# CESNET/GPUJPEG

Measured on AMD Instinct MI355X. Metric: Mpix/s encode+decode (8K RGB q75), higher is better.
Workload: dtype f32

## Files before the change

gpujpeg_amd/csrc/gj_enc_internal.h:

```cpp
#pragma once
#include <hip/hip_runtime.h>
#include <stdlib.h>

#include "gj_device.h"
#include "gj_hip.h"

#define GJ_ENC_MAX_SPT 64
#define GJ_ASM_SEGS 4

template <int CS_FROM, int CS_TO>
__device__ __forceinline__ void gj_color_static(int& a, int& b, int& c)
{
    if (CS_FROM == CS_TO || CS_FROM == GJ_CS_NONE || CS_TO == GJ_CS_NONE) return;
    if (CS_FROM == GJ_CS_RGB) gj_rgb_to(CS_TO, a, b, c);
    else if (CS_TO == GJ_CS_RGB) gj_to_rgb(CS_FROM, a, b, c);
}

template <int R0 = 0, int R1 = 8>
__device__ __forceinline__ void gj_load_444(const gj_geom& g, const uint8_t* __restrict__ raw, const unsigned bx, const unsigned by, uint32_t (&px)[8][6])
{
    const size_t pitch = (size_t)g.width * 3 + g.width_padding;
    const bool interior = (bx * 8 + 8 <= (unsigned)g.width) && (by * 8 + 8 <= (unsigned)g.height);
    const bool aligned = ((pitch | (size_t)raw) & 3) == 0;
    if (interior && aligned) {
        const uint8_t* row = raw + (size_t)(by * 8 + R0) * pitch + (size_t)bx * 24;
#pragma unroll
        for (int r = R0; r < R1; r++) {
            const uint2* p = reinterpret_cast<const uint2*>(row);
            const uint2 a = p[0], b = p[1], c = p[2];
            px[r][0] = a.x; px[r][1] = a.y; px[r][2] = b.x; px[r][3] = b.y; px[r][4] = c.x; px[r][5] = c.y;
            row += pitch;
        }
    } else {
#pragma unroll
        for (int r = R0; r < R1; r++) {
            const unsigned y = by * 8 + r;
#pragma unroll
            for (int w = 0; w < 6; w++) {
                uint32_t d = 0;
#pragma unroll
                for (int b = 0; b < 4; b++) {
                    const unsigned byte = w * 4 + b, x = bx * 8 + byte / 3;
                    if (x < (unsigned)g.width && y < (unsigned)g.height) d |= (uint32_t)raw[(size_t)y * pitch + (size_t)x * 3 + byte % 3] << (8 * b);
                }
                px[r][w] = d;
            }
        }
    }
}

template <int CS_FROM, int CS_TO>
__device__ __forceinline__ void gj_color_444(const gj_geom& g, const unsigned bx, const unsigned by, const uint32_t (&px)[8][6], uint32_t (&pk)[3][16])
{
    const bool interior = (bx * 8 + 8 <= (unsigned)g.width) && (by * 8 + 8 <= (unsigned)g.height);
#pragma unroll
    for (int r = 0; r < 8; r++) {
        uint32_t o0[2], o1[2], o2[2];
        gj_color_row<CS_FROM, CS_TO>(px[r], o0, o1, o2);
        if (!interior) {
            const int cols = min(8, max(0, g.width - (int)(bx * 8))), rows = min(8, max(0, g.height - (int)(by * 8)));
            const uint32_t m_lo = cols >= 4 ? 0xFFFFFFFFu : (1u << (8 * cols)) - 1u;
            const uint32_t m_hi = cols >= 8 ? 0xFFFFFFFFu : cols > 4 ? (1u << (8 * (cols - 4))) - 1u : 0u;
            const uint32_t lo = r < rows ? m_lo : 0u, hi = r < rows ? m_hi : 0u;
            o0[0] &= lo; o0[1] &= hi; o1[0] &= lo; o1[1] &= hi; o2[0] &= lo; o2[1] &= hi;
        }
        pk[0][r * 2] = o0[0]; pk[0][r * 2 + 1] = o0[1];
        pk[1][r * 2] = o1[0]; pk[1][r * 2 + 1] = o1[1];
        pk[2][r * 2] = o2[0]; pk[2][r * 2 + 1] = o2[1];
        GJ_KEEP6(pk[0][r * 2], pk[0][r * 2 + 1], pk[1][r * 2], pk[1][r * 2 + 1], pk[2][r * 2], pk[2][r * 2 + 1]);
    }
}

template <int CS_FROM, int CS_TO>
__device__ __forceinline__ void gj_load_color_444(const gj_geom& g, const uint8_t* __restrict__ raw, const unsigned bx, const unsigned by, uint32_t (&pk)[3][16])
{
    uint32_t px[8][6];
    gj_load_444(g, raw, bx, by, px);
    gj_color_444<CS_FROM, CS_TO>(g, bx, by, px, pk);
}


typedef uint32_t __attribute__((aligned(1))) gj_u32_unaligned;
struct GjTail {
    uint32_t* piece;
    uint32_t* group;
    uint32_t* group_other;
    uint32_t ngroups, npieces;
    const uint8_t* temp;
    const uint32_t* seg_bytes;
    const uint32_t* seg_ff;
    uint8_t* jpeg;
    uint64_t capacity;
    const uint8_t* scan_hdr;
    uint32_t hdr_end[GJ_MAX_COMP];
    uint32_t scan_first[GJ_MAX_COMP];
    uint32_t seg_first[GJ_MAX_COMP];
    uint32_t segs[GJ_MAX_COMP];
    uint32_t block_first[GJ_MAX_COMP];
    uint32_t spt, seg_blocks;
    uint64_t temp_blocks;
    uint32_t main_hdr;
    uint32_t* d_result;
    uint32_t* h_result;
    uint64_t f_raw, f_temp, f_jpeg;
    uint32_t f_seg, f_tail;
    uint32_t tail_from, tiles;
};

__device__ __forceinline__ uint32_t gj_pick4(const uint32_t (&a)[GJ_MAX_COMP], const uint32_t s)
{
    return s == 0 ? a[0] : s == 1 ? a[1] : s == 2 ? a[2] : a[3];
}
__device__ __forceinline__ uint32_t gj_tail_scan_of(const GjTail& T, const uint32_t p)
{
    return (p >= T.scan_first[1] ? 1u : 0u) + (p >= T.scan_first[2] ? 1u : 0u) + (p >= T.scan_first[3] ? 1u : 0u);
}
__device__ __forceinline__ void gj_piece_put(const GjTail& T, const uint32_t p, const uint32_t size, const size_t frame_words = 0)
{
    T.piece[frame_words + p] = size;
    (void)__hip_atomic_fetch_add(&T.group[frame_words + (p >> 5)], size, __ATOMIC_RELAXED, __HIP_MEMORY_SCOPE_AGENT);
}


typedef void (*gj_fused_kernel_t)(const gj_geom, const uint8_t*, int16_t*, const float*, const float*);
typedef void (*gj_encode_kernel_t)(const gj_geom, const uint8_t*, const float*, const float*, const uint32_t*, uint8_t*, uint32_t*, uint32_t*, const GjTail);
gj_fused_kernel_t gj_fused_kernel(const gj_geom& g);
gj_fused_kernel_t gj_fused_uyvy422_kernel();
gj_encode_kernel_t gj_encode_kernel(const gj_geom& g, const bool one_component = false);
gj_encode_kernel_t gj_encode_uyvy422_kernel();
gj_encode_kernel_t gj_encode_blocks_kernel(const bool planar);
__global__ void k_preprocess(const gj_geom g, const uint8_t* __restrict__ raw, uint8_t* __restrict__ planes);
__global__ void k_copy_planes_in(const gj_geom g, const uint8_t* __restrict__ raw, uint8_t* __restrict__ planes);
__global__ void k_dct(const gj_geom g, const uint8_t* __restrict__ planes, int16_t* __restrict__ coefs, const float* __restrict__ q_luma, const float* __restrict__ q_chroma);
__global__ void k_huffman(const gj_geom g, const int16_t* __restrict__ coefs, const uint32_t* __restrict__ lut, uint8_t* __restrict__ temp, uint32_t* __restrict__ seg_bytes,
                          uint32_t* __restrict__ seg_ff);
__global__ void k_huffman_count(const gj_geom g, const int16_t* __restrict__ coefs, uint32_t* __restrict__ freq);
__global__ void k_gather(const GjTail T0);
__global__ void k_scan_segments(const gj_enc_job J, unsigned long long* __restrict__ partial, const uint32_t epoch);
__global__ void k_assemble(const gj_enc_job J);
__global__ void k_segment_info(const gj_enc_job J);
```

gpujpeg_amd/csrc/gj_enc_tiles.hip:

```cpp
#include "gj_enc_internal.h"

#ifdef GJ_TRACE_PHASES
static __device__ unsigned long long* gj_trace_buf_e;
extern "C" GJ_HIP_API int gj_hip_trace_set_encoder(void* p) { return hipMemcpyToSymbol(HIP_SYMBOL(gj_trace_buf_e), &p, sizeof p) == hipSuccess ? 0 : -1; }
static __device__ int gj_trace_stop_e = 1 << 30;
extern "C" GJ_HIP_API int gj_hip_trace_stop_encoder(int n) { return hipMemcpyToSymbol(HIP_SYMBOL(gj_trace_stop_e), &n, sizeof n) == hipSuccess ? 0 : -1; }
#define GJ_TRACE_E(slot) do { if (threadIdx.x == 0 && gj_trace_buf_e) gj_trace_buf_e[(size_t)blockIdx.x * 16 + (slot)] = __builtin_amdgcn_s_memrealtime(); \
                              if ((slot) >= gj_trace_stop_e) __builtin_amdgcn_endpgm(); } while (0)
#else
#define GJ_TRACE_E(slot) ((void)0)
#endif

#define GJ_ENC_PRIV_ROWS 24
#define GJ_ENC_WIN_DW ((32 - GJ_ENC_PRIV_ROWS) * 256)

__device__ static constexpr uint8_t GJ_IZZ[64] = {0,  1,  5,  6,  14, 15, 27, 28, 2,  4,  7,  13, 16, 26, 29, 42, 3,  8,  12, 17, 25, 30,
                                                  41, 43, 9,  11, 18, 24, 31, 40, 44, 53, 10, 19, 23, 32, 39, 45, 52, 54, 20, 22, 33, 38,
                                                  46, 51, 55, 60, 21, 34, 37, 47, 50, 56, 59, 61, 35, 36, 48, 49, 57, 58, 62, 63};
#define GJ_COL_OFF(z) (((z) & 31) * 1024 + ((z) >> 5) * 2)

__device__ __forceinline__ void gj_fdct_quant_zz(const uint32_t (&px)[16], const float* __restrict__ q, uint8_t* col)
{
    gj_f2 D[8][4];
#pragma unroll
    for (int r = 0; r < 8; r++) {
        const uint32_t a = px[2 * r], b = px[2 * r + 1];
        D[r][0] = gj_f2{gj_ubyte_f_opaque<0>(a), gj_ubyte_f_opaque<1>(a)};
        D[r][1] = gj_f2{gj_ubyte_f_opaque<2>(a), gj_ubyte_f_opaque<3>(a)};
        D[r][2] = gj_f2{gj_ubyte_f_opaque<0>(b), gj_ubyte_f_opaque<1>(b)};
        D[r][3] = gj_f2{gj_ubyte_f_opaque<2>(b), gj_ubyte_f_opaque<3>(b)};
    }
#pragma unroll
    for (int c = 0; c < 4; c++) gj_fdct8<gj_f2>(D[0][c], D[1][c], D[2][c], D[3][c], D[4][c], D[5][c], D[6][c], D[7][c], -1024.0f);
    __builtin_amdgcn_sched_barrier(0);
    const gj_f2* q2 = reinterpret_cast<const gj_f2*>(q);
#pragma unroll
    for (int rp = 0; rp < 4; rp++) {
        gj_f2 E[8];
#pragma unroll
        for (int cp = 0; cp < 4; cp++) {
            E[2 * cp] = gj_f2{D[2 * rp][cp].x, D[2 * rp + 1][cp].x};
            E[2 * cp + 1] = gj_f2{D[2 * rp][cp].y, D[2 * rp + 1][cp].y};
        }
        gj_fdct8<gj_f2>(E[0], E[1], E[2], E[3], E[4], E[5], E[6], E[7], 0.0f);
#pragma unroll
        for (int j = 0; j < 8; j++) {
            const gj_f2 u = E[j] * q2[j * 4 + rp] + (gj_f2)12582912.0f;
            const float fx = u.x, fy = u.y;
            *reinterpret_cast<uint16_t*>(col + GJ_COL_OFF(GJ_IZZ[(2 * rp) * 8 + j])) = (uint16_t)__builtin_bit_cast(uint32_t, fx);
            *reinterpret_cast<uint16_t*>(col + GJ_COL_OFF(GJ_IZZ[(2 * rp + 1) * 8 + j])) = (uint16_t)__builtin_bit_cast(uint32_t, fy);
        }
        __builtin_amdgcn_sched_barrier(0);
    }
}

struct GjCoderLds {
    uint32_t* coef;
    const uint32_t* lut;
    uint32_t* wsum;
    int* edge;
    uint32_t *segx, *segend, *segbase, *segbits, *segff;
};

struct GjWalk {
    uint32_t hi;
    int room;
    int produced;
    int stored;
    int lim;
};
#define GJ_ENC_NO_STORE 4096

__device__ __forceinline__ void gj_put(GjWalk& w, const uint32_t cw, const int n, uint8_t* col, uint32_t* __restrict__ spill, const int p)
{
    w.room -= n;
    const uint64_t t = (uint64_t)cw << w.room;
    w.hi |= (uint32_t)(t >> 32);
    if (w.room <= 32) {
        if (w.lim <= min(p, GJ_ENC_PRIV_ROWS - 1)) {
            *reinterpret_cast<uint16_t*>(col + w.produced * 2048) = (uint16_t)(w.hi >> 16);
            *reinterpret_cast<uint16_t*>(col + w.produced * 2048 + 1024) = (uint16_t)w.hi;
            w.lim += 2;
        } else {
            if (w.lim != GJ_ENC_NO_STORE) w.stored = w.produced;
            spill[w.produced] = w.hi;
            w.lim = GJ_ENC_NO_STORE;
        }
        w.produced++;
        w.hi = (uint32_t)t;
        w.room += 32;
    }
}

template <bool NONZERO>
__device__ __forceinline__ void gj_value_bits2(const int v, int& nbits, uint32_t& bits)
{
    const int s = v >> 31, t = v + s;
    if (NONZERO) {
        nbits = 32 - gj_ffbh_i32(t);
    } else {
        const uint32_t a = (uint32_t)(t ^ s) | 1u;
        nbits = v ? 32 - __builtin_clz(a) : 0;
    }
    bits = __builtin_amdgcn_ubfe((uint32_t)t, 0, (uint32_t)nbits);
}

__device__ __forceinline__ void gj_walk_ac(uint8_t* col, const uint32_t mlo, const uint32_t mhi, const uint32_t* lut_ac, GjWalk& w,
                                           uint32_t* __restrict__ spill)
{
    int prev = 0;
#pragma unroll
    for (int half = 0; half < 2; half++) {
        uint32_t m = half ? mhi : mlo;
        while (m) {
            const int b = __builtin_ctz(m), p = b + 32 * half;
            m &= m - 1;
            int run = p - prev - 1;
            prev = p;
            const int v = *reinterpret_cast<const int16_t*>(col + b * 1024 + half * 2);
            if (run >= 16) {
                const uint32_t zrl = lut_ac[0xF0];
                do {
                    gj_put(w, zrl & 0x03FFFFFFu, (int)(zrl >> 26), col, spill, p);
                    run -= 16;
                } while (run >= 16);
            }
            const int sg = v >> 31, t = v + sg, k = gj_ffbh_i32(t);
            const uint32_t bits = __builtin_amdgcn_ubfe((uint32_t)t, 0, (uint32_t)(32 - k));
            const uint32_t ent = (lut_ac - 16)[gj_lshl_add_u32<4>((uint32_t)run, (uint32_t)k)];
            gj_put(w, (ent & 0x03FFFFFFu) | bits, (int)(ent >> 26), col, spill, p);
        }
    }
    if (prev != 63) {
        const uint32_t eob = lut_ac[0];
        gj_put(w, eob & 0x03FFFFFFu, (int)(eob >> 26), col, spill, 63);
    }
}

template <bool WHOLE>
__device__ __forceinline__ void gj_merge_stream(const GjWalk& w, const uint8_t* col, const uint32_t* __restrict__ spill, const uint64_t tail,
                                                const int ndw, const uint32_t sh, const uint32_t d0, uint32_t* s_bits, const uint32_t wbase,
                                                const uint32_t wend)
{
    uint32_t prevv = 0, d = d0;
    auto emit = [&](const uint32_t cur) {
        const uint32_t out = __builtin_amdgcn_alignbit(prevv, cur, sh);
        if (out && (WHOLE || (d >= wbase && d < wend))) atomicOr(&s_bits[d - wbase], out);
        prevv = cur;
        d++;
    };
    const int stored = w.lim == GJ_ENC_NO_STORE ? w.stored : w.produced;
    for (int f = 0; f < stored; f++)
        emit(((uint32_t)*reinterpret_cast<const uint16_t*>(col + f * 2048) << 16) | *reinterpret_cast<const uint16_t*>(col + f * 2048 + 1024));
    for (int f = stored; f < w.produced; f++) emit(spill[f]);
    emit((uint32_t)(tail >> 32));
    if (ndw > w.produced) emit((uint32_t)tail);
    if (ndw > w.produced + 1) emit(0u);
}

__device__ __forceinline__ uint32_t gj_code_tile(const GjCoderLds& L, const int i, const int j, const int k, const bool active, const int spt,
                                                 const int nblocks, const int table, const int dc_dist, const int seg_count_left,
                                                 uint8_t* __restrict__ region,
                                                 uint32_t* __restrict__ seg_bytes, uint32_t* __restrict__ seg_ff, const uint32_t first_segment,
                                                 const int trace0 = -1)
{
    (void)trace0;
    const int lane = i & 63, wave = i >> 6;
    uint8_t* const col = reinterpret_cast<uint8_t*>(L.coef) + i * 4;
    uint32_t* const s_bits = L.coef + GJ_ENC_PRIV_ROWS * 256;
    const uint32_t* const lut_ac = L.lut + table * 272;
    const uint32_t* const lut_dc = lut_ac + 256;

    uint32_t mlo = 0, mhi = 0;
    int dc = 0;
    {
        uint32_t elo = 0, ehi = 0;
#pragma unroll
        for (int q = 0; q < 32; q++) {
            const uint32_t d = L.coef[q * 256 + i];
            if (q == 0) dc = (int)(int16_t)(d & 0xFFFFu);
            const uint32_t m = gj_pk_min_u16(d, 0x00010001u);
            if (q < 16) elo |= m << q;
            else ehi |= m << (q - 16);
        }
        if (active) {
            mlo = __builtin_amdgcn_perm(ehi, elo, 0x05040100u);
            mhi = __builtin_amdgcn_perm(ehi, elo, 0x07060302u);
        }
    }
    if (lane >= 48) L.edge[wave * 16 + (lane - 48)] = dc;
    if (i < GJ_ENC_MAX_SPT) L.segff[i] = 0;
    __syncthreads();

    GjWalk w = {0, 64, 0, 0, 1};
    uint32_t* const spill = reinterpret_cast<uint32_t*>(region + (size_t)i * GJ_TEMP_BYTES_PER_BLOCK);
    int dc_diff = 0;
    {
        const int src = lane - dc_dist;
        int pred = __builtin_amdgcn_ds_bpermute((src & 63) << 2, dc);
        if (src < 0 && wave > 0) pred = L.edge[(wave - 1) * 16 + (16 + src)];
        if (k - dc_dist < 0) pred = 0;
        dc_diff = dc - pred;
    }
    if (active) {
        int nbits;
        uint32_t bits;
        gj_value_bits2<false>(dc_diff, nbits, bits);
        const uint32_t ent = lut_dc[nbits];
        gj_put(w, (ent & 0x03FFFFFFu) | bits, (int)(ent >> 26), col, spill, 0);
        gj_walk_ac(col, mlo & ~1u, mhi, lut_ac, w, spill);
    }
    const int fill = 64 - w.room;
    const uint32_t len = (uint32_t)w.produced * 32u + (uint32_t)fill;

    if (trace0 >= 0) GJ_TRACE_E(trace0 + 1);
    const uint32_t winc = gj_wave_incl_scan(len);
    if (lane == 63) L.wsum[wave] = winc;
    __syncthreads();
    uint32_t excl;
    {
        const uint32_t a = L.wsum[0], b = L.wsum[1], c = L.wsum[2];
        const uint32_t incl = winc + (wave == 0 ? 0u : wave == 1 ? a : wave == 2 ? a + b : a + b + c);
        if (active && k == 0) L.segx[j] = incl - len;
        if (active && k == nblocks - 1) L.segend[j] = incl;
        excl = incl - len;
    }
    {
        uint4* z = reinterpret_cast<uint4*>(s_bits) + i * 2;
        z[0] = make_uint4(0, 0, 0, 0);
        z[1] = make_uint4(0, 0, 0, 0);
    }
    __syncthreads();
    if (trace0 >= 0) GJ_TRACE_E(trace0 + 2);
    uint32_t sbits = 0, sdw = 0;
    if (lane < spt && lane < seg_count_left) {
        sbits = L.segend[lane] - L.segx[lane];
        sbits += (8u - (sbits & 7u)) & 7u;
        sdw = (sbits + 31u) >> 5;
    }
    const uint32_t sbase_incl = gj_wave_incl_scan(sdw);
    const uint32_t sbase = sbase_incl - sdw;
    const uint32_t total_dw = (uint32_t)__builtin_amdgcn_readlane((int)sbase_incl, 63);
    if (wave == 0) {
        if (lane < spt) { L.segbase[lane] = sbase; L.segbits[lane] = sbits; }
        if (lane == 63) L.segbase[spt] = total_dw;
    }
    uint32_t start_bit = 0;
    int pad_bits = 0;
    {
        const uint32_t my_base = (uint32_t)__builtin_amdgcn_ds_bpermute(j << 2, (int)sbase);
        const uint32_t my_x = active ? L.segx[j] : 0u;
        start_bit = my_base * 32u + (excl - my_x);
        if (active && k == nblocks - 1) pad_bits = (int)((8u - ((start_bit + len) & 7u)) & 7u);
    }

    const uint32_t sh = start_bit & 31u, d0 = start_bit >> 5;
    uint64_t tail = (uint64_t)w.hi << 32;
    if (pad_bits) tail |= (uint64_t)((1u << pad_bits) - 1u) << (64 - fill - pad_bits);
    const int ndw = w.produced + (fill + pad_bits > 32 ? 2 : (fill + pad_bits > 0 ? 1 : 0));
    const int nseg = min(spt, seg_count_left);
    uint32_t* const dst = reinterpret_cast<uint32_t*>(region);
    for (uint32_t wbase = 0; wbase < total_dw; wbase += GJ_ENC_WIN_DW) {
        const uint32_t wend = min(total_dw, wbase + (uint32_t)GJ_ENC_WIN_DW);
        if (wbase) {
            __syncthreads();
            for (uint32_t d = i; d < wend - wbase; d += 256) s_bits[d] = 0;
            __syncthreads();
        }
        if (active && d0 + (uint32_t)ndw + 1u > wbase && d0 < wend) {
            if (total_dw <= (uint32_t)GJ_ENC_WIN_DW) gj_merge_stream<true>(w, col, spill, tail, ndw, sh, d0, s_bits, 0u, total_dw);
            else gj_merge_stream<false>(w, col, spill, tail, ndw, sh, d0, s_bits, wbase, wend);
        }
        __syncthreads();
        for (int sl = wave; sl < nseg; sl += 4) {
            const uint32_t sb = L.segbase[sl], nfl = (L.segbits[sl] + 31u) >> 5;
            const uint32_t lo = max(sb, wbase), hi = min(sb + nfl, wend);
            uint32_t ffc = 0;
            for (uint32_t d = lo + (uint32_t)lane; d < hi; d += 64) {
                const uint32_t v = s_bits[d - wbase];
                ffc += (uint32_t)__builtin_popcount(((v & 0x7F7F7F7Fu) + 0x01010101u) & v & 0x80808080u);
                dst[d] = __builtin_bswap32(v);
            }
            ffc = gj_wave_incl_scan(ffc);
            if (lane == 63 && ffc) L.segff[sl] += ffc;
        }
    }
    __syncthreads();
    if (trace0 >= 0) GJ_TRACE_E(trace0 + 3);
    uint32_t out = 0;
    if (lane < nseg) {
        const uint32_t nb = (L.segbits[lane] + 7u) >> 3, ff = L.segff[lane];
        out = nb + ff + (lane != seg_count_left - 1 ? 2u : 0u);
        if (wave == 0) {
            seg_bytes[first_segment + lane] = nb;
            seg_ff[first_segment + lane] = ff;
        }
    }
    return (uint32_t)__builtin_amdgcn_readlane((int)gj_wave_incl_scan(out), 63);
}

__device__ __forceinline__ void gj_load_coder_lut(uint32_t* s_lut, const uint32_t* __restrict__ lut, const int i)
{
    static_assert(GJ_CODER_LUT_WORDS == 2 * 272 && GJ_CODER_LUT_WORDS % 4 == 0, "layout of GjCoderLds::lut");
    if (i < GJ_CODER_LUT_WORDS / 4) reinterpret_cast<uint4*>(s_lut)[i] = reinterpret_cast<const uint4*>(lut + GJ_CODER_LUT_OFFSET)[i];
}


template <int CS_FROM, int CS_TO, bool ONE_COMPONENT = false>
__global__ __launch_bounds__(256, 4) void k_encode_rgb444(const gj_geom g, const uint8_t* __restrict__ raw, const float* __restrict__ q_luma,
                                                          const float* __restrict__ q_chroma, const uint32_t* __restrict__ lut,
                                                          uint8_t* __restrict__ temp, uint32_t* __restrict__ seg_bytes,
                                                          uint32_t* __restrict__ seg_ff, const GjTail T)
{
    __shared__ __attribute__((aligned(16))) uint32_t s_coef[32 * 256];
    __shared__ __attribute__((aligned(8))) float s_q[3][64];
    __shared__ __attribute__((aligned(16))) uint32_t s_lut[2 * 272];
    __shared__ uint32_t s_wsum[4];
    __shared__ int s_edge[64];
    __shared__ uint32_t s_segx[GJ_ENC_MAX_SPT], s_segend[GJ_ENC_MAX_SPT], s_segbase[GJ_ENC_MAX_SPT + 1], s_segbits[GJ_ENC_MAX_SPT], s_segff[GJ_ENC_MAX_SPT];
    const GjCoderLds L = {s_coef, s_lut, s_wsum, s_edge, s_segx, s_segend, s_segbase, s_segbits, s_segff};

    const int i = threadIdx.x;
    GJ_TRACE_E(0);
    gj_load_coder_lut(s_lut, lut, i);
    if (i < 192) s_q[i >> 6][i & 63] = (g.comp[i >> 6].type ? q_chroma : q_luma)[i & 63];
    const size_t fz = blockIdx.z;
    raw += fz * T.f_raw;
    temp += fz * T.f_temp;
    seg_bytes += fz * T.f_seg;
    seg_ff += fz * T.f_seg;

    const gj_comp_geom& k0 = g.comp[0];
    const int B = g.seg_blocks;
    const int spt = 256 / B;
    const int tile_blocks = spt * B;
    const uint32_t recip = (65536u + (uint32_t)B - 1u) / (uint32_t)B;
    const int j = min((int)(((uint32_t)i * recip) >> 16), GJ_ENC_MAX_SPT - 1);
    const int k = i - j * B;
    unsigned tile = blockIdx.x, ntiles = gridDim.x;
    int only = ONE_COMPONENT ? (int)blockIdx.y : -1;
    if (!ONE_COMPONENT && T.tail_from != 0xFFFFFFFFu) {
        ntiles = T.tiles;
        if (blockIdx.x >= T.tail_from) {
            const unsigned r = blockIdx.x - T.tail_from, q = r / 3u;
            tile = T.tail_from + q;
            only = (int)(r - 3u * q);
        }
    }
    const int seg0 = (int)tile * spt;
    const unsigned nb = (unsigned)(k0.blocks_x * k0.blocks_y);
    const unsigned lb = tile * (unsigned)tile_blocks + (unsigned)i;
    const bool active = i < tile_blocks && lb < nb;
    unsigned bx, by;
    {
        const unsigned bxn = (unsigned)k0.blocks_x, lbc = min(lb, nb - 1u);
        if (bxn >= 256u) {
            const unsigned lb0 = tile * (unsigned)tile_blocks;
            const unsigned by0 = (unsigned)__builtin_amdgcn_readfirstlane((int)(lb0 / bxn));
            bx = lbc - by0 * bxn;
            by = by0;
            if (bx >= bxn) { bx -= bxn; by++; }
        } else {
            by = lbc / bxn;
            bx = lbc - by * bxn;
        }
    }

    uint32_t pk[3][16];
    gj_load_color_444<CS_FROM, CS_TO>(g, raw, bx, by, pk);
    __syncthreads();
    GJ_TRACE_E(1);

#pragma unroll
    for (int c = 0; c < 3; c++) {
        if (only >= 0 && c != only) continue;
        const gj_comp_geom& kc = g.comp[c];
#pragma unroll
        for (int t = 0; t < 16; t++) GJ_KEEP(pk[c][t]);
        gj_fdct_quant_zz(pk[c], s_q[c], reinterpret_cast<uint8_t*>(s_coef) + i * 4);
        GJ_TRACE_E(2 + 4 * c);
        const uint64_t first_block = kc.data_offset / 64 + (uint64_t)seg0 * B;
        const uint32_t size = gj_code_tile(L, i, j, k, active, spt, active ? min(B, (int)nb - (seg0 + j) * B) : 0, kc.type, 1, k0.segment_count - seg0,
                                           temp + first_block * GJ_TEMP_BYTES_PER_BLOCK, seg_bytes, seg_ff, (uint32_t)(kc.first_segment + seg0), 2 + 4 * c);
        if (i == 0) gj_piece_put(T, (uint32_t)c * ntiles + tile, size, fz * T.f_tail);
    }
}

__global__ __launch_bounds__(256, 4) void k_encode_uyvy422(const gj_geom g, const uint8_t* __restrict__ raw, const float* __restrict__ q_luma,
                                                           const float* __restrict__ q_chroma, const uint32_t* __restrict__ lut,
                                                           uint8_t* __restrict__ temp, uint32_t* __restrict__ seg_bytes,
                                                           uint32_t* __restrict__ seg_ff, const GjTail T)
{
    __shared__ __attribute__((aligned(16))) uint32_t s_coef[32 * 256];
    __shared__ __attribute__((aligned(8))) float s_q[2][64];
    __shared__ __attribute__((aligned(16))) uint32_t s_lut[2 * 272];
    __shared__ uint32_t s_wsum[4];
    __shared__ int s_edge[64];
    __shared__ uint32_t s_segx[GJ_ENC_MAX_SPT], s_segend[GJ_ENC_MAX_SPT], s_segbase[GJ_ENC_MAX_SPT + 1], s_segbits[GJ_ENC_MAX_SPT], s_segff[GJ_ENC_MAX_SPT];
    const GjCoderLds L = {s_coef, s_lut, s_wsum, s_edge, s_segx, s_segend, s_segbase, s_segbits, s_segff};

    const int i = threadIdx.x;
    gj_load_coder_lut(s_lut, lut, i);
    if (i < 128) s_q[i >> 6][i & 63] = (i < 64 ? q_luma : q_chroma)[i & 63];
    raw += (size_t)blockIdx.z * T.f_raw;
    temp += (size_t)blockIdx.z * T.f_temp;
    seg_bytes += (size_t)blockIdx.z * T.f_seg;
    seg_ff += (size_t)blockIdx.z * T.f_seg;

    const gj_comp_geom& kc = g.comp[1];
    const int ri = g.restart_interval;
    const int B = g.seg_blocks;
    const int spt = 256 / B;
    const int tile_blocks = spt * B;
    const uint32_t recip = (65536u + (uint32_t)B - 1u) / (uint32_t)B;
    const int j = min((int)(((uint32_t)i * recip) >> 16), GJ_ENC_MAX_SPT - 1);
    const int k = i - j * B;
    const int p = k & 3;
    const int seg0 = blockIdx.x * spt;
    const unsigned m = (unsigned)(seg0 + j) * (unsigned)ri + (unsigned)(k >> 2);
    const unsigned nm = (unsigned)g.mcu_count;
    const bool active = i < tile_blocks && seg0 + j < g.segment_count && m < nm;
    const unsigned my = m / (unsigned)kc.blocks_x, mx = m - my * (unsigned)kc.blocks_x;

    uint32_t px[16];
    {
        const size_t pitch = (size_t)g.width * 2 + g.width_padding;
        const bool interior = (mx * 16 + 16 <= (unsigned)g.width) && (my * 8 + 8 <= (unsigned)g.height);
        const bool aligned = ((pitch | (size_t)raw) & 15) == 0;
        if (!active) {
#pragma unroll
            for (int t = 0; t < 16; t++) px[t] = 0;
        } else if (interior && aligned) {
            const uint4* src = reinterpret_cast<const uint4*>(raw + (size_t)(my * 8) * pitch + (size_t)mx * 32);
            const size_t pitch4 = pitch >> 4;
            const int first = p == 1;
            const uint32_t selc = p == 2 ? 0x05040100u : 0x07060302u;
            uint4 lo[8], hi[8];
#pragma unroll
            for (int r = 0; r < 8; r++) {
                lo[r] = src[r * pitch4 + first];
                hi[r] = src[r * pitch4 + 1];
            }
#pragma unroll
            for (int r = 0; r < 8; r++) {
                const uint32_t y0 = __builtin_amdgcn_perm(lo[r].y, lo[r].x, 0x07050301u), y1 = __builtin_amdgcn_perm(lo[r].w, lo[r].z, 0x07050301u);
                const uint32_t uv01 = __builtin_amdgcn_perm(lo[r].y, lo[r].x, 0x06020400u), uv23 = __builtin_amdgcn_perm(lo[r].w, lo[r].z, 0x06020400u);
                const uint32_t uv45 = __builtin_amdgcn_perm(hi[r].y, hi[r].x, 0x06020400u), uv67 = __builtin_amdgcn_perm(hi[r].w, hi[r].z, 0x06020400u);
                const uint32_t c0 = __builtin_amdgcn_perm(uv23, uv01, selc), c1 = __builtin_amdgcn_perm(uv67, uv45, selc);
                px[2 * r] = p < 2 ? y0 : c0;
                px[2 * r + 1] = p < 2 ? y1 : c1;
            }
        } else {
#pragma unroll
            for (int r = 0; r < 8; r++) {
                const unsigned y = my * 8 + r;
                uint32_t d[2] = {0, 0};
#pragma unroll
                for (int t = 0; t < 8; t++) {
                    uint32_t v = 0;
                    if (y < (unsigned)g.height) {
                        if (p < 2) {
                            const unsigned x = mx * 16 + p * 8 + t;
                            if (x < (unsigned)g.width) v = raw[(size_t)y * pitch + (size_t)x * 2 + 1];
                        } else {
                            const unsigned cx = mx * 8 + t;
                            if (cx < (unsigned)kc.width) v = raw[(size_t)y * pitch + (size_t)cx * 4 + (p == 2 ? 0 : 2)];
// ... 223 lines not shown
```

gpujpeg_amd/csrc/gj_encode.hip:

```cpp
#include "gj_enc_internal.h"

static GjTail gj_make_tail(const gj_enc_job* job, const unsigned pieces, const unsigned (&scan_first)[GJ_MAX_COMP], const unsigned spt)
{
    const gj_geom& g = job->g;
    GjTail T;
    for (int s = 0; s < GJ_MAX_COMP; s++) {
        T.scan_first[s] = scan_first[s];
        T.hdr_end[s] = job->scan_hdr_offset[s + 1];
        const bool own_scan = !g.interleaved && s < g.comp_count;
        T.seg_first[s] = own_scan ? (uint32_t)g.comp[s].first_segment : 0u;
        T.segs[s] = own_scan ? (uint32_t)g.comp[s].segment_count : (uint32_t)g.segment_count;
        T.block_first[s] = own_scan ? (uint32_t)(g.comp[s].data_offset / 64) : 0u;
    }
    T.spt = spt;
    T.seg_blocks = (uint32_t)g.seg_blocks;
    const unsigned ngcap = GJ_TAIL_GROUPS_CAP(g.segment_count);
    T.group = job->d_tail + (job->tail_set & 1) * ngcap;
    T.group_other = job->d_tail + ((job->tail_set + 1) & 1) * ngcap;
    T.ngroups = (pieces + 31) / 32;
    T.piece = job->d_tail + 2 * ngcap;
    T.npieces = pieces;
    T.temp = job->d_temp;
    T.temp_blocks = (uint64_t)g.block_count;
    T.seg_bytes = job->d_seg_bytes;
    T.seg_ff = job->d_seg_ff;
    T.jpeg = job->d_jpeg;
    T.capacity = job->jpeg_capacity;
    T.scan_hdr = job->d_scan_hdr;
    T.main_hdr = job->main_hdr_size;
    T.d_result = job->d_result;
    T.h_result = job->h_result;
    const bool batch = job->batch.count > 1;
    T.f_raw = batch ? job->batch.raw : 0;
    T.f_temp = batch ? job->batch.temp : 0;
    T.f_jpeg = batch ? job->batch.jpeg : 0;
    T.f_seg = batch ? job->batch.seg : 0;
    T.f_tail = batch ? job->batch.tail : 0;
    return T;
}


static int gj_blocks_kernel_mode(const gj_geom& g)
{
    if (g.no_transform) return 1;
    if (g.pixel_format != GJ_PF_444_P012 || g.comp_count != 3) return -1;
    const int from = g.color_space, to = g.color_space_internal;
    const bool none = from == to || from == GJ_CS_NONE || to == GJ_CS_NONE;
    if (!none && !(from == GJ_CS_RGB && (to == GJ_CS_BT601 || to == GJ_CS_BT601_256 || to == GJ_CS_BT709))) return -1;
    return 0;
}

static bool gj_is_uyvy_layout(const gj_enc_job* job)
{
    const gj_geom& g = job->g;
    return job->use_fused && g.pixel_format == GJ_PF_422_P1020 && g.comp_count == 3 && g.no_transform == 0 &&
           (g.color_space == g.color_space_internal || g.color_space == GJ_CS_NONE || g.color_space_internal == GJ_CS_NONE) &&
           g.comp[0].samp_h == 2 && g.comp[0].samp_v == 1 && g.comp[1].samp_h == 1 && g.comp[1].samp_v == 1 && g.comp[2].samp_h == 1 &&
           g.comp[2].samp_v == 1 && g.comp[0].blocks_x == 2 * g.comp[1].blocks_x && g.comp[0].blocks_y == g.comp[1].blocks_y &&
           g.comp[2].blocks_x == g.comp[1].blocks_x && g.comp[2].blocks_y == g.comp[1].blocks_y;
}
static int gj_tile_kernel(const gj_enc_job* job)
{
    const gj_geom& g = job->g;
    if (job->stage != GJ_ENC_STAGE_ALL) return 0;
    const bool segs_ok = g.restart_interval > 0 && g.seg_blocks <= 256 && g.seg_blocks >= 256 / GJ_ENC_MAX_SPT;
    gj_encode_kernel_t whole = (job->use_fused && !job->keep_coefs) ? gj_encode_kernel(g) : nullptr;
    if (whole && job->tune.enc_by_blocks > 0 && gj_blocks_kernel_mode(g) == 0) whole = nullptr;
    if (gj_is_uyvy_layout(job) && !job->keep_coefs && g.interleaved && segs_ok && g.blocks_per_mcu == 4 && g.mcu_count == g.comp[1].blocks_x * g.comp[1].blocks_y &&
        g.comp[1].type == g.comp[2].type && !job->tune.enc_no_whole422)
        return 1;
    if (!whole && job->use_fused && !job->keep_coefs && segs_ok && gj_blocks_kernel_mode(g) >= 0) return 2;
    return whole ? 3 : 0;
}

extern "C" int gj_hip_encode_batchable(const gj_enc_job* job)
{
    return job->use_fused && !job->keep_coefs && !job->channel_remap && !job->flipped && !job->segment_info && gj_tile_kernel(job) != 0;
}

extern "C" int gj_hip_encode_tiles(const gj_enc_job* job) { return gj_tile_kernel(job) != 0; }

extern "C" int gj_hip_encode(const gj_enc_job* job, gj_stream_t stream, gj_event_t ev[GJ_ENC_EVENTS])
{
    hipStream_t st = (hipStream_t)stream;
    const gj_geom& g = job->g;
    if (g.blocks_per_mcu > GJ_MAX_MCU_BLOCKS) return -1;
    const unsigned frames = job->batch.count > 1 ? job->batch.count : 1u;
    if (frames > 1 && (!gj_hip_encode_batchable(job) || frames > 65535u)) return -1;
    if (job->stage != GJ_ENC_STAGE_ALL && (frames > 1 || (job->stage == GJ_ENC_STAGE_COUNT && !job->d_huff_freq))) return -1;
    gj_hip_note_reset();
    const bool code_only = job->stage == GJ_ENC_STAGE_CODE;
    if (ev && !code_only) GJ_HIP_CHECK(hipEventRecord((hipEvent_t)ev[0], st));
    if (job->channel_remap && !code_only) {
        const unsigned n = (unsigned)g.width * (unsigned)g.height;
        hipLaunchKernelGGL(k_channel_remap, dim3((n + 255) / 256), dim3(256), 0, st, g, const_cast<uint8_t*>(job->d_raw), job->channel_remap & 0xFFFFu);
    }
    bool tiles = true;
    GjTail T;
    T.npieces = 0;
    const int tile_kernel = gj_tile_kernel(job);
    gj_encode_kernel_t whole = tile_kernel == 3 ? gj_encode_kernel(g) : nullptr;
    gj_fused_kernel_t fused = job->use_fused ? gj_fused_kernel(g) : nullptr;
    const bool uyvy = gj_is_uyvy_layout(job);
    if (tile_kernel == 1) {
        if (ev) GJ_HIP_CHECK(hipEventRecord((hipEvent_t)ev[1], st));
        if (ev) GJ_HIP_CHECK(hipEventRecord((hipEvent_t)ev[2], st));
        const int spt = 256 / g.seg_blocks;
        const unsigned wgs = ((unsigned)g.segment_count + spt - 1) / spt;
        T = gj_make_tail(job, wgs, {0u, ~0u, ~0u, ~0u}, (unsigned)spt);
        hipLaunchKernelGGL(gj_encode_uyvy422_kernel(), dim3(wgs, 1, frames), dim3(256), 0, st, g, job->d_raw, job->d_fwd_q[0], job->d_fwd_q[1], job->d_huff_lut,
                           job->d_temp, job->d_seg_bytes, job->d_seg_ff, T);
    } else if (tile_kernel == 2) {
        if (ev) GJ_HIP_CHECK(hipEventRecord((hipEvent_t)ev[1], st));
        if (ev) GJ_HIP_CHECK(hipEventRecord((hipEvent_t)ev[2], st));
        const int spt = 256 / g.seg_blocks;
        unsigned wgs = 0, scan_first[GJ_MAX_COMP] = {0u, ~0u, ~0u, ~0u};
        if (g.interleaved) wgs = ((unsigned)g.segment_count + spt - 1) / spt;
        else
            for (int c = 0; c < g.comp_count; c++) {
                scan_first[c] = wgs;
// ... 81 lines not shown
```

gpujpeg_amd/csrc/gj_runtime.hip:

```cpp
#include <hip/hip_runtime.h>
#include <stdlib.h>
#include <string.h>

#include <cstdio>
#include <cstring>
#include <mutex>

#include "gj_hip.h"

static thread_local hipError_t g_last = hipSuccess;

static int chk(hipError_t e)
{
    if (e != hipSuccess) {
        g_last = e;
        return -1;
    }
    return 0;
}

extern "C" {

int gj_hip_note(int hip_error) { return chk((hipError_t)hip_error); }
void gj_hip_note_reset(void) { g_last = hipSuccess; }
// ... 87 lines not shown
static hipStream_t g_lane[64][2];
static int g_lanes_enabled = 1;
static void gj_lanes_forget(int dev)
{
    std::lock_guard<std::mutex> lk(g_lane_mutex);
    if (dev >= 0 && dev < 64) g_lane[dev][0] = g_lane[dev][1] = nullptr;
}
static hipStream_t gj_lane(int dir, size_t n)
{
    int dev = 0;
    if (hipGetDevice(&dev) != hipSuccess || dev < 0 || dev >= 64) return nullptr;
    std::lock_guard<std::mutex> lk(g_lane_mutex);
    if (!g_lanes_enabled || n < g_lane_min_bytes) return nullptr;
    if (!g_lane[dev][dir] && hipStreamCreateWithFlags(&g_lane[dev][dir], hipStreamNonBlocking) != hipSuccess) {
        (void)hipGetLastError();
        g_lane[dev][dir] = nullptr;
    }
    return g_lane[dev][dir];
}
int gj_hip_upload(void* d, const void* s, size_t n, gj_stream_t st, gj_event_t done)
{
    hipStream_t lane = done ? gj_lane(0, n) : nullptr;
    if (!lane) return chk(hipMemcpyAsync(d, s, n, hipMemcpyHostToDevice, (hipStream_t)st));
    if (chk(hipMemcpyAsync(d, s, n, hipMemcpyHostToDevice, lane)) || chk(hipEventRecord((hipEvent_t)done, lane))) return -1;
    return chk(hipEventSynchronize((hipEvent_t)done));
}
int gj_hip_download(void* d, const void* s, size_t n, gj_stream_t st, gj_event_t done)
{
    hipStream_t lane = done ? gj_lane(1, n) : nullptr;
    if (!lane) return chk(hipMemcpyAsync(d, s, n, hipMemcpyDeviceToHost, (hipStream_t)st));
    if (chk(hipStreamSynchronize((hipStream_t)st))) return -1;
    if (chk(hipMemcpyAsync(d, s, n, hipMemcpyDeviceToHost, lane)) || chk(hipEventRecord((hipEvent_t)done, lane))) return -1;
    return chk(hipEventSynchronize((hipEvent_t)done));
}
gj_stream_t gj_hip_lane_begin(int download, size_t bytes_each, gj_stream_t st)
{
    hipStream_t lane = gj_lane(download ? 1 : 0, bytes_each);
    if (!lane) return st;
    if (download && chk(hipStreamSynchronize((hipStream_t)st))) return st;
    return (gj_stream_t)lane;
}
int gj_hip_lane_end(gj_stream_t lane, gj_stream_t st, gj_event_t done)
{
    if (lane == st) return 0;
    if (chk(hipEventRecord((hipEvent_t)done, (hipStream_t)lane))) return -1;
    return chk(hipEventSynchronize((hipEvent_t)done));
}
int gj_hip_memset(void* d, int v, size_t n, gj_stream_t st) { return chk(hipMemsetAsync(d, v, n, (hipStream_t)st)); }
int gj_hip_stream_sync(gj_stream_t st) { return chk(hipStreamSynchronize((hipStream_t)st)); }

int gj_hip_is_device_ptr(const void* p)
{
    hipPointerAttribute_t a;
    std::memset(&a, 0, sizeof a);
    if (hipPointerGetAttributes(&a, p) != hipSuccess) {
        (void)hipGetLastError();
        return 0;
    }
    return a.type == hipMemoryTypeDevice ? 1 : 0;
}

gj_event_t gj_hip_event_create(void)
{
    hipEvent_t e = nullptr;
    if (chk(hipEventCreate(&e))) return nullptr;
    return (gj_event_t)e;
}
void gj_hip_event_destroy(gj_event_t e)
{
    if (e) (void)hipEventDestroy((hipEvent_t)e);
}
int gj_hip_event_record(gj_event_t e, gj_stream_t s) { return chk(hipEventRecord((hipEvent_t)e, (hipStream_t)s)); }
float gj_hip_event_elapsed_ms(gj_event_t a, gj_event_t b)
{
    float ms = 0.0f;
    if (hipEventSynchronize((hipEvent_t)b) != hipSuccess) return 0.0f;
    if (hipEventElapsedTime(&ms, (hipEvent_t)a, (hipEvent_t)b) != hipSuccess) return 0.0f;
    return ms;
}

}

static std::mutex g_tune_mutex;
static gj_tuning g_tune = { 0,  -1,  -1, 0, 0, 0, 0,  -1, 0, 0, 0, 0, 0, 0, 0, 0, 0, 0, 0, 0, 0};
static const char* const g_tune_names[] = {"GPUJPEG_NO_FUSED", "GPUJPEG_HOST_SCAN", "GJ_ENC_NO_WHOLE422", "GJ_DEC_TOKENS", "GJ_DEC_NO_TOKENS", "GJ_DEC_ENTROPY", "GJ_DEC_G",
                                           "GJ_DEC_SUB", "GJ_DEC_NO_SPEC", "GJ_DEC_SEQ", "GJ_DEC_DEBUG_SYNC", "GJ_DEC_TOK_NOCOOP", "GJ_SCAN_SHAPE", "GJ_ENC_BLOCKS",
                                           "GJ_HOST_TIMING", "GJ_DEC_BALANCE", "GJ_ENC_SPLIT", "GJ_ENC_TAIL", "GJ_DEC_FILL", "GJ_ENC_OUT_CAP", "GJ_IDCT_DENSE", "GJ_COPY_LANES", nullptr};
static bool gj_tune_apply(gj_tuning* t, const char* name, const char* v)
{
    const auto is = [&](const char* n) { return std::strcmp(name, n) == 0; };
    const int num = std::atoi(v);
    if (is("GPUJPEG_NO_FUSED")) t->no_fused = 1;
    else if (is("GPUJPEG_HOST_SCAN")) t->host_scan = 1;
    else if (is("GJ_ENC_NO_WHOLE422")) t->enc_no_whole422 = 1;
    else if (is("GJ_DEC_TOKENS")) { if (v[0] == '1') t->dec_tokens = 1; }
    else if (is("GJ_DEC_NO_TOKENS")) t->dec_tokens = 0;
    else if (is("GJ_DEC_ENTROPY")) t->dec_serial = v[0] == 's';
    else if (is("GJ_DEC_G")) t->dec_batch = num;
    else if (is("GJ_DEC_SUB")) t->dec_sub = num;
    else if (is("GJ_DEC_NO_SPEC")) t->dec_no_spec = 1;
    else if (is("GJ_DEC_SEQ")) t->dec_seq = v[0] == '1' ? 1 : 2;
    else if (is("GJ_DEC_DEBUG_SYNC")) t->debug_sync = v[0] == '1';
    else if (is("GJ_DEC_TOK_NOCOOP")) t->dec_tok_nocoop = v[0] == '1';
    else if (is("GJ_SCAN_SHAPE")) t->scan_shape = num;
    else if (is("GJ_ENC_BLOCKS")) t->enc_by_blocks = num;
    else if (is("GJ_HOST_TIMING")) t->host_timing = v[0] == '1';
    else if (is("GJ_DEC_BALANCE")) t->dec_balance = v[0] == '1';
    else if (is("GJ_ENC_SPLIT")) t->enc_split = num;
    else if (is("GJ_ENC_TAIL")) t->enc_tail = num;
    else if (is("GJ_DEC_FILL")) t->dec_fill = num;
    else if (is("GJ_ENC_OUT_CAP")) t->enc_out_cap = num;
    else if (is("GJ_IDCT_DENSE")) t->idct_dense = v[0] == '1';
    else if (is("GJ_COPY_LANES")) {
        std::lock_guard<std::mutex> lk(g_lane_mutex);
        g_lanes_enabled = !(v[0] == '0' && v[1] == 0);
        g_lane_min_bytes = num > 0 ? (size_t)num << 20 : (size_t)1 << 20;
    } else return false;
    return true;
}
extern "C" int gj_hip_tuning_setting(const char* setting)
{
    std::lock_guard<std::mutex> lk(g_tune_mutex);
    if (setting == nullptr) {
        g_tune = gj_tuning{0, -1, -1, 0, 0, 0, 0, -1, 0, 0, 0, 0, 0, 0, 0, 0, 0, 0, 0, 0, 0};
        std::lock_guard<std::mutex> lk2(g_lane_mutex);
        g_lanes_enabled = 1;
        g_lane_min_bytes = (size_t)1 << 20;
        return 0;
    }
    char name[40];
    const char* eq = std::strchr(setting, '=');
    const size_t n = eq ? (size_t)(eq - setting) : std::strlen(setting);
    if (n == 0 || n >= sizeof name) return -1;
    std::memcpy(name, setting, n);
    name[n] = 0;
    return gj_tune_apply(&g_tune, name, eq ? eq + 1 : "") ? 0 : -1;
}
extern "C" const char* const* gj_hip_tuning_names(int* count)
{
    *count = (int)(sizeof g_tune_names / sizeof g_tune_names[0]) - 1;
    return g_tune_names;
}
extern "C" void gj_hip_tuning_defaults(gj_tuning* t)
{
    {
        std::lock_guard<std::mutex> lk(g_tune_mutex);
        *t = g_tune;
    }
#ifdef GJ_TUNING_ENV
    for (const char* n : g_tune_names)
        if (n != nullptr)
            if (const char* e = getenv(n)) gj_tune_apply(t, n, e);
#endif
}
```

include/gj_hip.h:

```cpp
#ifndef GJ_HIP_H
#define GJ_HIP_H

#include <stddef.h>
#include <stdint.h>

#ifdef __cplusplus
extern "C" {
#endif

#define GJ_HIP_API __attribute__((visibility("default")))

typedef void* gj_stream_t;
typedef void* gj_event_t;

GJ_HIP_API int gj_hip_device_count(void);
GJ_HIP_API int gj_hip_get_device(int* device);
GJ_HIP_API int gj_hip_set_device(int device);
GJ_HIP_API int gj_hip_device_reset(void);
GJ_HIP_API int gj_hip_device_props(int device, char name[256], int* major, int* minor, size_t* global_mem, size_t* shared_mem,
                        int* regs_per_block, int* cu_count);
GJ_HIP_API int gj_hip_cu_count(void);
GJ_HIP_API int gj_hip_runtime_version(int* driver, int* runtime);
GJ_HIP_API const char* gj_hip_last_error(void);

// ... 16 lines not shown
GJ_HIP_API void gj_hip_event_destroy(gj_event_t e);
GJ_HIP_API int gj_hip_event_record(gj_event_t e, gj_stream_t s);
GJ_HIP_API float gj_hip_event_elapsed_ms(gj_event_t start, gj_event_t stop);

#define GJ_MAX_COMP 4
#define GJ_MAX_MCU_BLOCKS 16
#define GJ_TEMP_BYTES_PER_BLOCK 208
#define GJ_TAIL_GROUPS_CAP(segments) (((unsigned)(segments) + 32u) / 32u + 1u)
#define GJ_TAIL_WORDS(segments) (2u * GJ_TAIL_GROUPS_CAP(segments) + ((unsigned)(segments) + 1u))

enum { GJ_PF_U8 = 0, GJ_PF_444_P012 = 1, GJ_PF_444_P0P1P2 = 2, GJ_PF_422_P1020 = 3, GJ_PF_422_P0P1P2 = 4,
       GJ_PF_420_P0P1P2 = 5, GJ_PF_4444_P0123 = 6 };

typedef struct gj_comp_geom {
    int type;
    int samp_h, samp_v;
    int sub_h, sub_v;
    int width, height;
    int data_width, data_height;
    int blocks_x, blocks_y;
    int mcu_count_x, mcu_count;
    int segment_count;
    int first_segment;
    int q_table, dc_table, ac_table;
    int reserved;
    uint64_t data_offset;
} gj_comp_geom;

typedef struct gj_frame_strides {
    const uint32_t* sizes;
    uint64_t jpeg, raw;
    uint64_t coefs, tok, rec;
    uint32_t seg;
    uint32_t frames;
} gj_frame_strides;

typedef struct gj_geom {
    int width, height, width_padding;
    int pixel_format, color_space, color_space_internal;
    int comp_count, interleaved, restart_interval;
    int max_h, max_v;
    int mcu_count;
    int mcu_count_x;
    int segment_count;
    int scan_count;
    int blocks_per_mcu;
    int seg_blocks;
    int block_count;
    int raw_width;
    int no_transform;
    uint64_t data_size;
    uint64_t raw_size;
    gj_comp_geom comp[GJ_MAX_COMP];
    uint8_t mcu_comp[GJ_MAX_MCU_BLOCKS];
    uint8_t mcu_bx[GJ_MAX_MCU_BLOCKS];
    uint8_t mcu_by[GJ_MAX_MCU_BLOCKS];
    uint8_t mcu_prev[GJ_MAX_MCU_BLOCKS];
    gj_frame_strides fb;
} gj_geom;

#define GJ_CODER_LUT_OFFSET 1024
#define GJ_CODER_LUT_WORDS 544
typedef struct gj_tuning {
    int no_fused;
    int enc_split;
    int enc_tail;
    int dec_balance;
    int host_timing;
    int host_scan;
    int enc_no_whole422;
    int dec_tokens;
    int dec_serial;
    int dec_batch;
    int dec_sub;
    int dec_no_spec;
    int dec_seq;
    int debug_sync;
    int scan_shape;
    int dec_tok_nocoop;
    int enc_by_blocks;
    int dec_fill;
    int enc_out_cap;
    int idct_dense;
    int dec_careful;
} gj_tuning;
GJ_HIP_API void gj_hip_tuning_defaults(gj_tuning* t);
GJ_HIP_API int gj_hip_tuning_setting(const char* setting);
GJ_HIP_API const char* const* gj_hip_tuning_names(int* count);

typedef struct gj_batch {
    uint32_t count;
    uint64_t raw;
    uint64_t jpeg;
    uint64_t temp;
    uint64_t coefs;
    uint64_t tok;
    uint64_t rec;
    uint32_t seg;
    uint32_t tail;
    uint32_t scratch;
    uint32_t maxlen;
    const uint32_t* d_sizes;
} gj_batch;

typedef struct gj_enc_job {
    gj_geom g;
    const uint8_t* d_raw;
    uint8_t* d_planes;
    int16_t* d_coefs;
    const float* d_fwd_q[2];
    const uint32_t* d_huff_lut;
    uint8_t* d_temp;
    uint32_t* d_seg_bytes;
    uint32_t* d_seg_ff;
    uint32_t* d_seg_out;
    uint8_t* d_jpeg;
    uint64_t jpeg_capacity;
    uint32_t* d_result;
    uint32_t* h_result;
    uint32_t* d_tail;
    int tail_set;
    uint64_t* d_scan_partial;
    uint32_t epoch;
    gj_tuning tune;
    const uint8_t* d_scan_hdr;
    uint32_t scan_hdr_offset[GJ_MAX_COMP + 1];
    uint32_t scan_info_payload[GJ_MAX_COMP];
    uint32_t main_hdr_size;
    int segment_info;
    int use_fused;
    int keep_coefs;
    int flipped;
    uint32_t channel_remap;
    gj_batch batch;
    int stage;
    uint32_t* d_huff_freq;
} gj_enc_job;
enum { GJ_ENC_STAGE_ALL = 0, GJ_ENC_STAGE_COUNT = 1, GJ_ENC_STAGE_CODE = 2 };
GJ_HIP_API int gj_hip_encode_batchable(const gj_enc_job* job);
GJ_HIP_API int gj_hip_encode_tiles(const gj_enc_job* job);

#define GJ_ENC_EVENTS 8
GJ_HIP_API int gj_hip_encode(const gj_enc_job* job, gj_stream_t stream, gj_event_t ev[GJ_ENC_EVENTS]);


struct gj_scan_summary;
typedef struct gj_scan_deferred {
    int valid;
    uint32_t wgs, part_bytes;
    uint64_t begin, size;
    const uint32_t* recs;
    const uint32_t* lists;
    uint32_t* d_seg_pos;
    uint32_t* d_seg_len;
    uint32_t* d_seg_index;
    uint32_t max_segments;
    struct gj_scan_summary* d_summary;
    struct gj_scan_summary* h_summary;
    uint32_t* h_maxlen_parts;
    uint32_t maxlen_capacity;
    uint32_t* maxlen_part_count;
    int* folded;
} gj_scan_deferred;

typedef struct gj_region_frame {
    int x, y;
// ... 112 lines not shown
```

Measured before the change: 175,700.

## Add chroma corner fast path skipping full quantized coefficient scan when high frequencies vanish

For chroma components, the forward DCT row pass now quantizes only the low-frequency 4x4 corner into shared memory. It also tracks the maximum magnitude of the remaining coefficients. If a whole wave has no high-frequency coefficient that rounds to nonzero, the entropy coder reuses the nonzero mask and DC gathered during quantization instead of rescanning all 64 coefficients. Otherwise it redoes the row pass normally, and later chroma components skip the trial once it fails. This is meant to cut the per-block mask/scan cost for smooth chroma, at the price of extra work on waves where the trial fails.

Result: no change. 176,600 (median of 6 runs) (+0.6%).

```diff
diff --git a/gpujpeg_amd/csrc/gj_enc_internal.h b/gpujpeg_amd/csrc/gj_enc_internal.h
--- a/gpujpeg_amd/csrc/gj_enc_internal.h
+++ b/gpujpeg_amd/csrc/gj_enc_internal.h
@@ -105,6 +105,7 @@
     uint64_t f_raw, f_temp, f_jpeg;
     uint32_t f_seg, f_tail;
     uint32_t tail_from, tiles;
+    uint32_t enc_dense;
 };
 
 __device__ __forceinline__ uint32_t gj_pick4(const uint32_t (&a)[GJ_MAX_COMP], const uint32_t s)
diff --git a/gpujpeg_amd/csrc/gj_enc_tiles.hip b/gpujpeg_amd/csrc/gj_enc_tiles.hip
--- a/gpujpeg_amd/csrc/gj_enc_tiles.hip
+++ b/gpujpeg_amd/csrc/gj_enc_tiles.hip
@@ -19,9 +19,8 @@
                                                   46, 51, 55, 60, 21, 34, 37, 47, 50, 56, 59, 61, 35, 36, 48, 49, 57, 58, 62, 63};
 #define GJ_COL_OFF(z) (((z) & 31) * 1024 + ((z) >> 5) * 2)
 
-__device__ __forceinline__ void gj_fdct_quant_zz(const uint32_t (&px)[16], const float* __restrict__ q, uint8_t* col)
-{
-    gj_f2 D[8][4];
+__device__ __forceinline__ void gj_fdct_cols_zz(const uint32_t (&px)[16], gj_f2 (&D)[8][4])
+{
 #pragma unroll
     for (int r = 0; r < 8; r++) {
         const uint32_t a = px[2 * r], b = px[2 * r + 1];
@@ -33,16 +32,24 @@
 #pragma unroll
     for (int c = 0; c < 4; c++) gj_fdct8<gj_f2>(D[0][c], D[1][c], D[2][c], D[3][c], D[4][c], D[5][c], D[6][c], D[7][c], -1024.0f);
     __builtin_amdgcn_sched_barrier(0);
-    const gj_f2* q2 = reinterpret_cast<const gj_f2*>(q);
+}
+
+__device__ __forceinline__ void gj_fdct_row_pair(const gj_f2 (&D)[8][4], const int rp, gj_f2 (&E)[8])
+{
+#pragma unroll
+    for (int cp = 0; cp < 4; cp++) {
+        E[2 * cp] = gj_f2{D[2 * rp][cp].x, D[2 * rp + 1][cp].x};
+        E[2 * cp + 1] = gj_f2{D[2 * rp][cp].y, D[2 * rp + 1][cp].y};
+    }
+    gj_fdct8<gj_f2>(E[0], E[1], E[2], E[3], E[4], E[5], E[6], E[7], 0.0f);
+}
+
+__device__ __forceinline__ void gj_fdct_rows_zz(const gj_f2 (&D)[8][4], const gj_f2* q2, uint8_t* col)
+{
 #pragma unroll
     for (int rp = 0; rp < 4; rp++) {
         gj_f2 E[8];
-#pragma unroll
-        for (int cp = 0; cp < 4; cp++) {
-            E[2 * cp] = gj_f2{D[2 * rp][cp].x, D[2 * rp + 1][cp].x};
-            E[2 * cp + 1] = gj_f2{D[2 * rp][cp].y, D[2 * rp + 1][cp].y};
-        }
-        gj_fdct8<gj_f2>(E[0], E[1], E[2], E[3], E[4], E[5], E[6], E[7], 0.0f);
+        gj_fdct_row_pair(D, rp, E);
 #pragma unroll
         for (int j = 0; j < 8; j++) {
             const gj_f2 u = E[j] * q2[j * 4 + rp] + (gj_f2)12582912.0f;
@@ -52,6 +59,77 @@
         }
         __builtin_amdgcn_sched_barrier(0);
     }
+}
+
+__device__ __forceinline__ void gj_fdct_quant_zz(const uint32_t (&px)[16], const float* __restrict__ q, uint8_t* col)
+{
+    gj_f2 D[8][4];
+    gj_fdct_cols_zz(px, D);
+    gj_fdct_rows_zz(D, reinterpret_cast<const gj_f2*>(q), col);
+}
+
+struct GjCorner {
+    uint32_t mask;
+    int dc;
+};
+
+template <bool TRIAL>
+__device__ __forceinline__ bool gj_fdct_quant_zz(const uint32_t (&px)[16], const float* __restrict__ q, uint8_t* col, const bool trial, GjCorner& K)
+{
+    gj_f2 D[8][4];
+    gj_fdct_cols_zz(px, D);
+    const gj_f2* q2 = reinterpret_cast<const gj_f2*>(q);
+    uint32_t q_again = 0;
+    if (TRIAL && trial) {
+        float mx = 0.0f;
+        uint32_t mask = 0;
+        int dc = 0;
+#pragma unroll
+        for (int t = 0; t < 4; t++) {
+            const int rp = 3 - t;
+            gj_f2 E[8];
+            gj_fdct_row_pair(D, rp, E);
+#pragma unroll
+            for (int j = 0; j < 8; j++) {
+                const gj_f2 P = E[j] * q2[j * 4 + rp];
+                if (rp < 2 && j < 4) {
+                    const gj_f2 u = P + (gj_f2)12582912.0f;
+                    const float fx = u.x, fy = u.y;
+                    const uint32_t bx = __builtin_bit_cast(uint32_t, fx), by = __builtin_bit_cast(uint32_t, fy);
+                    const int zx = GJ_IZZ[(2 * rp) * 8 + j], zy = GJ_IZZ[(2 * rp + 1) * 8 + j];
+                    *reinterpret_cast<uint16_t*>(col + GJ_COL_OFF(zx)) = (uint16_t)bx;
+                    *reinterpret_cast<uint16_t*>(col + GJ_COL_OFF(zy)) = (uint16_t)by;
+                    mask |= gj_pk_min_u16(bx, 1u) << zx;
+                    mask |= gj_pk_min_u16(by, 1u) << zy;
+                    if (rp == 0 && j == 0) dc = (int)(int16_t)(bx & 0xFFFFu);
+                } else {
+                    mx = __builtin_fmaxf(__builtin_fmaxf(__builtin_fabsf(P.x), __builtin_fabsf(P.y)), mx);
+                }
+            }
+            if (rp < 2) GJ_KEEP(mask);
+            __builtin_amdgcn_sched_barrier(0);
+        }
+        if (__ballot(mx > 0.5f) == 0ull) {
+            K.mask = mask;
+            K.dc = dc;
+            return true;
+        }
+#pragma unroll
+        for (int r = 0; r < 8; r++) {
+#pragma unroll
+            for (int c = 0; c < 4; c++) {
+                float a = D[r][c].x, b = D[r][c].y;
+                GJ_KEEP(a);
+                GJ_KEEP(b);
+                D[r][c] = gj_f2{a, b};
+            }
+        }
+        GJ_KEEP(q_again);
+        gj_fdct_rows_zz(D, q2 + q_again, col);
+        return false;
+    }
+    gj_fdct_rows_zz(D, q2, col);
+    return false;
 }
 
 struct GjCoderLds {
@@ -162,7 +240,7 @@
                                                  const int nblocks, const int table, const int dc_dist, const int seg_count_left,
                                                  uint8_t* __restrict__ region,
                                                  uint32_t* __restrict__ seg_bytes, uint32_t* __restrict__ seg_ff, const uint32_t first_segment,
-                                                 const int trace0 = -1)
+                                                 const int trace0 = -1, const bool corner = false, const GjCorner K = {0u, 0})
 {
     (void)trace0;
     const int lane = i & 63, wave = i >> 6;
@@ -173,7 +251,10 @@
 
     uint32_t mlo = 0, mhi = 0;
     int dc = 0;
-    {
+    if (corner) {
+        dc = K.dc;
+        if (active) mlo = K.mask;
+    } else {
         uint32_t elo = 0, ehi = 0;
 #pragma unroll
         for (int q = 0; q < 32; q++) {
@@ -306,6 +387,10 @@
 }
 
 
+#ifdef GJ_HIPEMU
+extern "C" GJ_HIP_API unsigned long long gj_emu_enc_corner_waves[2][2];
+unsigned long long gj_emu_enc_corner_waves[2][2] = {{0, 0}, {0, 0}};
+#endif
 template <int CS_FROM, int CS_TO, bool ONE_COMPONENT = false>
 __global__ __launch_bounds__(256, 4) void k_encode_rgb444(const gj_geom g, const uint8_t* __restrict__ raw, const float* __restrict__ q_luma,
                                                           const float* __restrict__ q_chroma, const uint32_t* __restrict__ lut,
@@ -371,17 +456,32 @@
     __syncthreads();
     GJ_TRACE_E(1);
 
+    bool try_corner = T.enc_dense == 0u;
 #pragma unroll
     for (int c = 0; c < 3; c++) {
         if (only >= 0 && c != only) continue;
         const gj_comp_geom& kc = g.comp[c];
 #pragma unroll
         for (int t = 0; t < 16; t++) GJ_KEEP(pk[c][t]);
-        gj_fdct_quant_zz(pk[c], s_q[c], reinterpret_cast<uint8_t*>(s_coef) + i * 4);
+        bool corner = false;
+        GjCorner K = {0u, 0};
+        int ic = i;
+        GJ_KEEP(ic);
+        __builtin_assume(ic >= 0 && ic < 256);
+        if (c == 0) {
+            gj_fdct_quant_zz(pk[c], s_q[c], reinterpret_cast<uint8_t*>(s_coef) + ic * 4);
+        } else {
+            corner = gj_fdct_quant_zz<true>(pk[c], s_q[c], reinterpret_cast<uint8_t*>(s_coef) + ic * 4, try_corner, K);
+            try_corner = corner;
+#ifdef GJ_HIPEMU
+            if ((i & 63) == 0) __atomic_fetch_add(&gj_emu_enc_corner_waves[c - 1][corner ? 1 : 0], 1ull, __ATOMIC_RELAXED);
+#endif
+        }
         GJ_TRACE_E(2 + 4 * c);
         const uint64_t first_block = kc.data_offset / 64 + (uint64_t)seg0 * B;
-        const uint32_t size = gj_code_tile(L, i, j, k, active, spt, active ? min(B, (int)nb - (seg0 + j) * B) : 0, kc.type, 1, k0.segment_count - seg0,
-                                           temp + first_block * GJ_TEMP_BYTES_PER_BLOCK, seg_bytes, seg_ff, (uint32_t)(kc.first_segment + seg0), 2 + 4 * c);
+        const uint32_t size = gj_code_tile(L, ic, j, k, active, spt, active ? min(B, (int)nb - (seg0 + j) * B) : 0, kc.type, 1, k0.segment_count - seg0,
+                                           temp + first_block * GJ_TEMP_BYTES_PER_BLOCK, seg_bytes, seg_ff, (uint32_t)(kc.first_segment + seg0), 2 + 4 * c,
+                                           corner, K);
         if (i == 0) gj_piece_put(T, (uint32_t)c * ntiles + tile, size, fz * T.f_tail);
     }
 }
diff --git a/gpujpeg_amd/csrc/gj_encode.hip b/gpujpeg_amd/csrc/gj_encode.hip
--- a/gpujpeg_amd/csrc/gj_encode.hip
+++ b/gpujpeg_amd/csrc/gj_encode.hip
@@ -36,6 +36,7 @@
     T.f_jpeg = batch ? job->batch.jpeg : 0;
     T.f_seg = batch ? job->batch.seg : 0;
     T.f_tail = batch ? job->batch.tail : 0;
+    T.enc_dense = job->tune.enc_dense ? 1u : 0u;
     return T;
 }
 
diff --git a/gpujpeg_amd/csrc/gj_runtime.hip b/gpujpeg_amd/csrc/gj_runtime.hip
--- a/gpujpeg_amd/csrc/gj_runtime.hip
+++ b/gpujpeg_amd/csrc/gj_runtime.hip
@@ -193,10 +193,10 @@
 }
 
 static std::mutex g_tune_mutex;
-static gj_tuning g_tune = { 0,  -1,  -1, 0, 0, 0, 0,  -1, 0, 0, 0, 0, 0, 0, 0, 0, 0, 0, 0, 0, 0};
+static gj_tuning g_tune = { 0,  -1,  -1, 0, 0, 0, 0,  -1, 0, 0, 0, 0, 0, 0, 0, 0, 0, 0, 0, 0, 0, 0};
 static const char* const g_tune_names[] = {"GPUJPEG_NO_FUSED", "GPUJPEG_HOST_SCAN", "GJ_ENC_NO_WHOLE422", "GJ_DEC_TOKENS", "GJ_DEC_NO_TOKENS", "GJ_DEC_ENTROPY", "GJ_DEC_G",
                                            "GJ_DEC_SUB", "GJ_DEC_NO_SPEC", "GJ_DEC_SEQ", "GJ_DEC_DEBUG_SYNC", "GJ_DEC_TOK_NOCOOP", "GJ_SCAN_SHAPE", "GJ_ENC_BLOCKS",
-                                           "GJ_HOST_TIMING", "GJ_DEC_BALANCE", "GJ_ENC_SPLIT", "GJ_ENC_TAIL", "GJ_DEC_FILL", "GJ_ENC_OUT_CAP", "GJ_IDCT_DENSE", "GJ_COPY_LANES", nullptr};
+                                           "GJ_HOST_TIMING", "GJ_DEC_BALANCE", "GJ_ENC_SPLIT", "GJ_ENC_TAIL", "GJ_DEC_FILL", "GJ_ENC_OUT_CAP", "GJ_IDCT_DENSE", "GJ_ENC_DENSE", "GJ_COPY_LANES", nullptr};
 static bool gj_tune_apply(gj_tuning* t, const char* name, const char* v)
 {
     const auto is = [&](const char* n) { return std::strcmp(name, n) == 0; };
@@ -222,6 +222,7 @@
     else if (is("GJ_DEC_FILL")) t->dec_fill = num;
     else if (is("GJ_ENC_OUT_CAP")) t->enc_out_cap = num;
     else if (is("GJ_IDCT_DENSE")) t->idct_dense = v[0] == '1';
+    else if (is("GJ_ENC_DENSE")) t->enc_dense = v[0] == '1';
     else if (is("GJ_COPY_LANES")) {
         std::lock_guard<std::mutex> lk(g_lane_mutex);
         g_lanes_enabled = !(v[0] == '0' && v[1] == 0);
@@ -233,7 +234,7 @@
 {
     std::lock_guard<std::mutex> lk(g_tune_mutex);
     if (setting == nullptr) {
-        g_tune = gj_tuning{0, -1, -1, 0, 0, 0, 0, -1, 0, 0, 0, 0, 0, 0, 0, 0, 0, 0, 0, 0, 0};
+        g_tune = gj_tuning{0, -1, -1, 0, 0, 0, 0, -1, 0, 0, 0, 0, 0, 0, 0, 0, 0, 0, 0, 0, 0, 0};
         std::lock_guard<std::mutex> lk2(g_lane_mutex);
         g_lanes_enabled = 1;
         g_lane_min_bytes = (size_t)1 << 20;
diff --git a/include/gj_hip.h b/include/gj_hip.h
--- a/include/gj_hip.h
+++ b/include/gj_hip.h
@@ -122,6 +122,7 @@
     int dec_fill;
     int enc_out_cap;
     int idct_dense;
+    int enc_dense;
     int dec_careful;
 } gj_tuning;
 GJ_HIP_API void gj_hip_tuning_defaults(gj_tuning* t);
```
